# mir-group/pair_allegro

Measured on AMD Instinct MI355X. Metric: atom_steps_per_sec, higher is better.
Workload: dtype f32-equivalent (f16x2 split on the f16 matrix cores, f32 accumulate); 1 GPU; BASELINE config 4: 1000000-atom bulk Si (50^3 diamond cells), model S (l_max=1, U=32, S=64, 2 layers), r_max 5.0 A + skin 1.0 A, NVE dt=1 fs; grid=1x1x1, rebuilds=4, comm=serial, comm_transport=library/hosted/single-rank gather-scatter

## Files before the change

pair_allegro_amd/csrc/fused.hip:

```cpp
#include <hip/hip_runtime.h>

#include <cmath>
#include <algorithm>
#include <cstdio>
#include <cstdlib>
#include <cstring>
#include <type_traits>

#include "../../include/allegro_hip.h"
#include "engine.h"
#define AHIP_RING 4
#include "fused_common.h"
#include "fused_h.h"
#include "prims.h"

#ifndef AHIP_FUSED_PART
#define AHIP_FUSED_PART 0
#endif
namespace ahip {


[[maybe_unused]] static constexpr int MAX_TILE_SLOTS = 128;
static constexpr int MAXNL = 3;
static constexpr int STG_LD = 132;
// ... 150 lines not shown
      } else { prev0 = acc0; prev1 = acc1; }
    }
    __builtin_amdgcn_sched_barrier(0);
  }
  wp += NS * 256;
  pin_s(wp);
}
template <int RB> __device__ __forceinline__ void ring_prime_b(__amdgpu_buffer_rsrc_t W, int wp, int v16, u32x4 (&ring)[RB]) {
  int wo = wp * 4;
  pin_s(wo);
#pragma unroll
  for (int j = 0; j < RB; ++j) ring[j] = __builtin_bit_cast(u32x4, bload_w(W, v16 + (j & 3) * 1024, wo + (j >> 2) * 4096));
}

template <int NW, int NL> __device__ __forceinline__ void reduce_stage(const Lds<NW, NL> &lds, const int *aoff, float *dst, int na, float scale, int tid) {
  const int fidx = tid & 127;
  for (int a = tid >> 7; a < na; a += NW / 2) {
    const int s0 = aoff[a], s1 = aoff[a + 1];
    float acc0 = 0.f, acc1 = 0.f, acc2 = 0.f, acc3 = 0.f;
    int sl = s0;
    for (; sl + 4 <= s1; sl += 4) {
      acc0 += lds.stage[sl * STG_LD + fidx];
      acc1 += lds.stage[(sl + 1) * STG_LD + fidx];
      acc2 += lds.stage[(sl + 2) * STG_LD + fidx];
      acc3 += lds.stage[(sl + 3) * STG_LD + fidx];
    }
    for (; sl < s1; ++sl) acc0 += lds.stage[sl * STG_LD + fidx];
    dst[a * ENV_LD + fidx] = scale * ((acc0 + acc1) + (acc2 + acc3));
  }
}
enum { PH_GEOM = 0, PH_TB, PH_EMB, PH_ENV, PH_TP, PH_MIX, PH_LAT, PH_OUT, PH_BLAT, PH_BMIX, PH_BTP, PH_BENV, PH_BEMB, PH_BTB, PH_FIN, PH_N };
#define PHASE(id) do { if (PROF) { long long _t = clock64(); pacc[id] += _t - tprev; tprev = _t; } } while (0)

template <int AR> struct RingT {
  int act = 1;
  f32x4 f[AR != 0 ? 1 : RING];
  u32x4 b[AR == 0 ? 1 : (AR == 1 ? RINGB : AR == 2 ? RINGB2 : RINGH)];
};
template <int AR, int KT, int NT, bool ACC, int RPI, class Epi>
__device__ __forceinline__ void lin(__amdgpu_buffer_rsrc_t W, int &wp, const f32x4 (&in)[KT], f32x4 (&out)[NT], int v16, RingT<AR> &ring, Epi epi) {
  if (!ring.act) {
    if constexpr (!ACC) {
#pragma unroll
      for (int t = 0; t < NT; ++t) out[t] = f32x4{0.f, 0.f, 0.f, 0.f};
    }
    return;
  }
  if constexpr (AR == 3) {
    static_assert(KT % 2 == 0, "K-steps are pairs of 16-feature tiles");
    Hop b[1][KT / 2], unused[1][NT / 2];
#pragma unroll
    for (int ks = 0; ks < KT / 2; ++ks) b[0][ks] = split_pair_h(in[2 * ks], in[2 * ks + 1]);
    Epi ep[1] = {epi};
    linear_h<1, KT / 2, NT, ACC, false, (4 * RPI) % RINGH, Epi>(W, wp, b, reinterpret_cast<f32x4 (&)[1][NT]>(out), unused, v16, ring.b, ep);
  } else if constexpr (AR != 0) {
    static_assert(KT % 2 == 0, "K-steps are pairs of 16-feature tiles");
    constexpr int NTERM = AR == 1 ? 3 : 2;
    Bop b[KT / 2], unused[NT / 2];
#pragma unroll
    for (int ks = 0; ks < KT / 2; ++ks) b[ks] = split_pair(in[2 * ks], in[2 * ks + 1]);
    linear_b<KT / 2, NT, ACC, false, (2 * NTERM * RPI) % RingB<NTERM>::N, Epi, NTERM>(W, wp, b, out, unused, v16, ring.b, epi);
  } else {
    linear_s<KT, NT, ACC, (4 * RPI) % RING, Epi>(W, wp, in, out, v16, ring.f, epi);
  }
}

template <int RPI, class Epi>
__device__ __forceinline__ void lin_m3(__amdgpu_buffer_rsrc_t W, int &wp, const f32x4 (&in0)[2], const f32x4 (&in1)[2], const f32x4 (&in2)[2], f32x4 (&out)[3][2], int v16,
                                       RingT<3> &ring, Epi (&epi)[3]) {
  if (!ring.act) {
#pragma unroll
    for (int q = 0; q < 3; ++q) { out[q][0] = f32x4{0.f, 0.f, 0.f, 0.f}; out[q][1] = f32x4{0.f, 0.f, 0.f, 0.f}; }
    return;
  }
  Hop b[3][1], unused[3][1];
  b[0][0] = split_pair_h(in0[0], in0[1]); b[1][0] = split_pair_h(in1[0], in1[1]); b[2][0] = split_pair_h(in2[0], in2[1]);
  linear_h<3, 1, 2, false, false, (4 * RPI) % RINGH, Epi>(W, wp, b, out, unused, v16, ring.b, epi);
}

struct TileIn {
  int a0, a1, e0, e1;
  float rx, ry, rz;
  int eii, jat, tt;
  int eoff;
};
__device__ __forceinline__ void tile_fetch(const FusedArgs &A, int tile, int ntiles, int s, int tid, TileIn &n) {
  n.a0 = n.a1 = n.e0 = n.e1 = 0;
  n.rx = 1.f; n.ry = 0.f; n.rz = 0.f;
  n.eii = 0; n.jat = 0; n.tt = 0; n.eoff = 0;
  if (tile >= ntiles) return;
  n.a0 = A.tile_a0[tile]; n.a1 = A.tile_a0[tile + 1]; n.e0 = A.tile_e0[tile]; n.e1 = A.tile_e0[tile + 1];
  const int e = n.e0 + s, na = n.a1 - n.a0;
  if (e < n.e1) {
    n.rx = A.rvec[3 * (size_t)e]; n.ry = A.rvec[3 * (size_t)e + 1]; n.rz = A.rvec[3 * (size_t)e + 2];
    n.eii = A.e_ii[e];
    n.jat = A.e_j[e];
    n.tt = A.e_tt[e];
  }
  if (tid <= na) n.eoff = A.eoff[n.a0 + tid];
}

template <int NW, bool PROF, int AR, bool TBT, int NLT, int MD = 2, bool VA = false>
__global__ void __launch_bounds__(NW * 64, 2) k_fused(FusedArgs A) {
  constexpr int NTHREADS = NW * 64, MAXA = Lds<NW>::MAXA;
  constexpr bool SAVEZ = AR == 3;
  constexpr bool PARKV = true;
  constexpr bool STGROWS = true;
  constexpr int OZL = 4 + 4 * (MD - 1), OU = 4 + 4 * MD, OVIN = 8 + 4 * MD;
  static_assert(MD >= 1 && MD <= 3 && (MD == 2 || (AR == 3 && TBT)), "latent MLP depth 1 / 3: f16x2 instances with the two-body table only");
  __shared__ Lds<NW, NLT> lds;
  const int tid = threadIdx.x, lane = tid & 63, j = lane & 15, g = lane >> 4, wave = tid >> 6;
  const int v16 = lane * 16;
  __amdgpu_buffer_rsrc_t SB, WB;
  {
    unsigned long long b = (unsigned long long)(A.scratch + (size_t)blockIdx.x * A.wg_scratch + (size_t)wave * A.wave_scratch);
    unsigned lo = __builtin_amdgcn_readfirstlane((unsigned)b), hi = __builtin_amdgcn_readfirstlane((unsigned)(b >> 32));
    SB = __builtin_amdgcn_make_buffer_rsrc((void *)(((unsigned long long)hi << 32) | lo), 0, (int)(A.wave_scratch * 4), 0x00020000);
    WB = __builtin_amdgcn_make_buffer_rsrc((void *)A.wbase, 0, A.wbytes, 0x00020000);
  }
  if (A.maxdeg_sel && ((*A.maxdeg_sel <= 64) != (NW == 4))) return;
  const float *__restrict__ Wb = A.wbase;
  for (int k = tid; k < A.NL * 160; k += NTHREADS) {
    const int pth = (k % 160) / 32;
    lds.tp[k / 160][k % 160] = Wb[A.o_tpl + k] * (pth == 1 ? C_P1 : pth == 4 ? C_P4 : 1.f);
  }
  const int ntiles = *A.ntiles;
  constexpr int NL = NLT;
  double acc_part = 0.0;
  long long pacc[PH_N];
  long long tprev = 0;
  const long long t_clk0 = clock64(), t_wall0 = wall_clock64();
  if (PROF) {
#pragma unroll
    for (int k = 0; k < PH_N; ++k) pacc[k] = 0;
    tprev = clock64();
  }
  float *const pk = lds.park[wave];
  RingT<AR> ring;
  int wp = A.o_stream;
  if constexpr (AR != 0) ring_prime_b(WB, wp, v16, ring.b);
  else ring_prime(WB, wp, v16, ring.f);
  if (tid < MAXA) lds.eacc[tid] = 0.0;
  if (lane < 6) lds.virw[wave][lane] = 0.0;
  if (A.T <= 4 && tid < A.T * A.T) lds.rc[tid] = (float)A.rcut[tid];
  if (tid < A.T) { lds.scale[tid] = Wb[A.o_scale + tid]; lds.shift[tid] = Wb[A.o_shift + tid]; }
  if (tid < 2 * A.NL) lds.res[tid >> 1][tid & 1] = Wb[A.o_res[tid >> 1] + (tid & 1)];

  const int s = wave * 16 + j;
  float *const st = lds.stage + s * STG_LD;
  if (tid == 0) lds.chunk[0] = (int)atomicAdd(A.tile_counter, (unsigned)A.tchunk);
  __syncthreads();
  int par = 0, cpar = 0, ck = 0;
  int cbase = __builtin_amdgcn_readfirstlane(lds.chunk[0]);

  TileIn nx_;
  tile_fetch(A, cbase, ntiles, s, tid, nx_);

  for (;;) {
    const int tile = cbase + ck;
    if (tile >= ntiles) break;
    int claimed = 0;
    if (ck == 0 && tid == 0) claimed = (int)atomicAdd(A.tile_counter, (unsigned)A.tchunk);
    const int a0 = nx_.a0, a1 = nx_.a1, e0 = nx_.e0, e1 = nx_.e1;
    const int wact = __builtin_amdgcn_readfirstlane(e0 + wave * 16 < e1 ? 1 : 0);
    ring.act = wact;
    const int v16t = wact ? v16 : 0x7ffffff0;
    const int na = a1 - a0;
    par ^= 1;
    int *const aoffp = lds.aoff[par];
    const int e = e0 + s;
    const bool valid = e < e1;
    const float rx = nx_.rx, ry = nx_.ry, rz = nx_.rz;
    const int aloc = valid ? nx_.eii - a0 : 0, jat = nx_.jat, ti = nx_.tt >> 4, tj = nx_.tt & 15;
    if (tid <= na) aoffp[tid] = nx_.eoff - e0;
    const float d = sqrtf(rx * rx + ry * ry + rz * rz);
    const float inv = 1.f / d;
    const float nx = rx * inv, ny = ry * inv, nz = rz * inv;
    const float rc = A.T <= 4 ? lds.rc[ti * A.T + tj] : (float)A.rcut[ti * A.T + tj];
    const float xx = d / rc;
    float fc, dfc_dx;
    cutoff_poly_c(A.p, A.cp, xx, fc, dfc_dx);
    if (!valid) { fc = 0.f; dfc_dx = 0.f; }
    const float Y1 = C_S3 * ny, Y2 = C_S3 * nz, Y3 = C_S3 * nx;
    const float pref = 2.f / rc;
    const float PI = 3.14159265358979323846f;
    const float *const envrow = lds.env[0] + aloc * ENV_LD;
    const float *const denvrow = lds.denv + aloc * ENV_LD;
    PHASE(PH_GEOM);

    f32x4 x[4];
    float tb_t = 0.f, tb_invh = 0.f;
    if constexpr (TBT) {
      tb_invh = (float)A.tb_nk / rc;
      const float sft = d * tb_invh;
      const int kq = min((int)sft, A.tb_nk - 1);
      tb_t = sft - (float)kq;
#ifdef ABL_NOTBGATHER
      const int tb_off = (A.o_tbtab + 4 * g) * 4;
#else
      const int tb_off = (A.o_tbtab + ((ti * A.T + tj) * A.tb_nk + kq) * 256 + 4 * g) * 4;
#endif
      const float vm = (valid && xx < 1.f) ? 1.f : 0.f;
#pragma unroll
      for (int t = 0; t < 4; ++t) {
        const f32x4 c0 = bload_w(WB, tb_off + (t * 4 + 0) * 64, 0), c1 = bload_w(WB, tb_off + (t * 4 + 1) * 64, 0);
        const f32x4 c2 = bload_w(WB, tb_off + (t * 4 + 2) * 64, 0), c3 = bload_w(WB, tb_off + (t * 4 + 3) * 64, 0);
        x[t] = (c0 + tb_t * (c1 + tb_t * (c2 + tb_t * c3))) * vm;
        bstore(SB, v16t, (R_Z1TB() + t) * ROW * 4, (c1 + tb_t * (2.f * c2 + (3.f * tb_t) * c3)) * (vm * tb_invh));
      }
    } else {
      f32x4 z[4], z2[4];
      {
        const float *pt = Wb + A.o_pair + (size_t)(ti * A.T + tj) * 64;
#pragma unroll
        for (int t = 0; t < 4; ++t) z[t] = *(const f32x4 *)(pt + 16 * t + 4 * g);
      }
      f32x4 bfin[2];
#pragma unroll
      for (int r = 0; r < 4; ++r) {
        const float n = (float)(4 * g + r + 1);
        bfin[0][r] = g < 2 ? pref * __builtin_amdgcn_sinf(0.5f * n * xx) * inv * fc : 0.f;
        bfin[1][r] = 0.f;
      }
      lin<AR, 2, 4, true, 0>(WB, wp, bfin, z, v16t, ring, EpiSiluSaveD{SB, R_Z1TB(), v16t});
      lin<AR, 4, 4, false, 0>(WB, wp, z, z2, v16t, ring, EpiSiluSaveD{SB, R_Z2TB(), v16t});
      lin<AR, 4, 4, false, 0>(WB, wp, z2, x, v16t, ring, EpiSaveScale{{SB, R_U0(), v16t}, fc});
    }
    PHASE(PH_TB);
    {
      f32x4 w0[4];
      lin<AR, 4, 4, false, 0>(WB, wp, x, w0, v16t, ring, EpiSavePark{{SB, R_W0(), v16t}, pk, 0, lane});
    }
    if (ck == 0 && tid == 0) lds.chunk[cpar ^ 1] = claimed;
// ... 95 lines not shown
          if (stg && (H) >= MD - 1) { \
            if (SAVEZ && (H) == MD) lin<AR, KT, 4, false, 0>(WB, wp, IN, OUT, v16t, ring, EpiSiluSaveZL{sq, 4}); \
            else lin<AR, KT, 4, false, 0>(WB, wp, IN, OUT, v16t, ring, EpiSiluSaveDL{sq, (H) == MD ? 4 : 0}); \
          } else if (SAVEZ && (H) == MD) lin<AR, KT, 4, false, 0>(WB, wp, IN, OUT, v16t, ring, EpiSiluSaveZ{SB, RL + 4 * (H), v16t}); \
          else lin<AR, KT, 4, false, 0>(WB, wp, IN, OUT, v16t, ring, EpiSiluSaveD{SB, RL + 4 * (H), v16t}); } while (0)
        AHIP_HIDDEN(6, cat, z, 1);
        if constexpr (MD >= 2) AHIP_HIDDEN(4, z, z2, 2);
        if constexpr (MD >= 3) AHIP_HIDDEN(4, z2, z, 3);
#undef AHIP_HIDDEN
        f32x4 (&zl)[4] = MD == 2 ? z2 : z;
        const float ra = lds.res[kk][0], rbf = lds.res[kk][1] * fc;
        if (!last) {
          f32x4 xn[4];
          if constexpr (SAVEZ) lin<AR, 4, 4, false, 0>(WB, wp, zl, xn, v16t, ring, EpiResidualNS<4>{x, ra, rbf});
          else lin<AR, 4, 4, false, 0>(WB, wp, zl, xn, v16t, ring, EpiResidual<4>{{SB, RL + OU, v16t}, x, ra, rbf});
          x[0] = xn[0]; x[1] = xn[1]; x[2] = xn[2]; x[3] = xn[3];
        } else {
          f32x4 za[2], up[2];
          if constexpr (SAVEZ) lin<AR, 4, 2, false, 0>(WB, wp, zl, up, v16t, ring, EpiNone{});
          else lin<AR, 4, 2, false, 0>(WB, wp, zl, up, v16t, ring, EpiSave{SB, RL + OU, v16t});
          lin<AR, 4, 2, false, 0>(WB, wp, x, za, v16t, ring, EpiNone{});
          zr[0] = ra * za[0] + rbf * up[0]; zr[1] = ra * za[1] + rbf * up[1];
        }
      }
      PHASE(PH_LAT);
    }

    f32x4 upre[4], zt[4], w0h[2];
#pragma unroll
    for (int t = 0; t < 2; ++t) if (!SAVEZ) upre[t] = bload(SB, v16t, (R_LAYER(NL - 1, MD) + OU + t) * ROW * 4);
    if (!STGROWS) load_rows<4>(SB, R_LAYER(NL - 1, MD) + OZL, zt, v16t);
    __builtin_amdgcn_sched_barrier(0);
    f32x4 wo1[2];
#pragma unroll
    for (int t = 0; t < 2; ++t) wo1[t] = *(const f32x4 *)(Wb + A.o_out1 + 16 * t + 4 * g);
    float eps = 0.f;
#pragma unroll
    for (int t = 0; t < 2; ++t)
#pragma unroll
      for (int r = 0; r < 4; ++r) eps += silu1(zr[t][r]) * wo1[t][r];
    eps = gsum(eps);
    asm volatile("" : "+v"(eps));

    float bsc = 1.f;
    if constexpr (AR == 3) {
      int bex;
      (void)frexpf(lds.scale[ti] * A.cenv, &bex);
      bex = min(max(bex, -100), 100);
      bsc = ldexpf(1.f, -bex);
      if (g == 0) st[128] = ldexpf(1.f, bex);
    }
    const float deps = valid ? lds.scale[ti] * A.cenv * bsc : 0.f;
    f32x4 dx[4];
    f32x4 dzr[2];
#pragma unroll
    for (int t = 0; t < 2; ++t)
#pragma unroll
      for (int r = 0; r < 4; ++r) dzr[t][r] = deps * wo1[t][r] * dsilu1(zr[t][r]);
    lin<AR, 2, 4, false, 0>(WB, wp, dzr, dx, v16t, ring, EpiNone{});
    if (STGROWS) {
#pragma unroll
      for (int t = 0; t < 4; ++t) zt[t] = stg_load(st + 4 * g, 4 + t);
    }
    float dfc_part = 0.f, dY1 = 0.f, dY2 = 0.f, dY3 = 0.f;
    PHASE(PH_OUT);

#pragma unroll
    for (int kk = NL - 1; kk >= 0; --kk) {
// ... 249 lines not shown
      const float inve = 1.f / sqrtf(rxe * rxe + rye * rye + rze * rze);
      const float nxe = rxe * inve, nye = rye * inve, nze = rze * inve;
      const float gn = Gx * nxe + Gy * nye + Gz * nze;
      const float gx = dd * nxe + (Gx - gn * nxe) * inve;
      const float gy = dd * nye + (Gy - gn * nye) * inve;
      const float gz = dd * nze + (Gz - gn * nze) * inve;
      if (A.dbg && valid && g == 0) {
        float *dp = A.dbg + 8 * (size_t)e;
        dp[0] = gx; dp[1] = gy; dp[2] = gz; dp[3] = dd; dp[4] = dfc_tot; dp[5] = y1; dp[6] = y2; dp[7] = y3;
      }
#if !defined(ABL_NOW) && !defined(ABL_NOROWS) && !defined(ABL_NOROWLD) && !defined(ABL_NOROWST)
      if (AR == 3 && valid && !(fabsf(gx) + fabsf(gy) + fabsf(gz) + fabsf(eps) < 3.0e38f)) *A.err = 1;
#endif
      if (g == 0) {
        st[0] = valid ? gx : 0.f; st[1] = valid ? gy : 0.f; st[2] = valid ? gz : 0.f; st[3] = valid ? eps : 0.f;
        if (valid) {
#ifndef ABL_NOATOM
          atomicAdd(&A.f[3 * (size_t)jat], -(double)gx);
          atomicAdd(&A.f[3 * (size_t)jat + 1], -(double)gy);
          atomicAdd(&A.f[3 * (size_t)jat + 2], -(double)gz);
#endif
        }
      }
      float w6[6] = {-rx * gx, -ry * gy, -rz * gz, -0.5f * (rx * gy + ry * gx), -0.5f * (rx * gz + rz * gx), -0.5f * (ry * gz + rz * gy)};
#pragma unroll
      for (int c = 0; c < 6; ++c) w6[c] = valid ? w6[c] : 0.f;
#pragma unroll
      for (int c = 0; c < 6; ++c) {
#pragma unroll
        for (int off = 8; off > 0; off >>= 1) w6[c] += __shfl_xor(w6[c], off, 64);
      }
      if (lane < 6) {
        const float mine = lane == 0 ? w6[0] : lane == 1 ? w6[1] : lane == 2 ? w6[2] : lane == 3 ? w6[3] : lane == 4 ? w6[4] : w6[5];
        lds.virw[wave][lane] += (double)mine;
      }
      if constexpr (VA) vatom_scatter(A.vatom, jat, g, valid, rx, ry, rz, gx, gy, gz);
    }
    int tidf = tid;
    asm volatile("" : "+v"(tidf));
    const int caf = tidf >> 4;
    int2 cil = make_int2(0, 0);
    if (caf < na) cil = A.centre[a0 + caf];
    __syncthreads();
    {
      const int col = tidf & 3, part = (tidf >> 2) & 3;
      float sum = 0.f;
      if (caf < na)
        for (int sl = aoffp[caf] + part; sl < aoffp[caf + 1]; sl += 4) sum += lds.stage[sl * STG_LD + col];
      sum += __shfl_xor(sum, 4, 64);
      sum += __shfl_xor(sum, 8, 64);
      if (caf < na && part == 0) {
        if (col < 3) atomicAdd(&A.f[3 * (size_t)cil.x + col], (double)sum);
        else {
          const float ei = lds.scale[cil.y] * (sum * A.cenv) + lds.shift[cil.y];
          if (A.eatom) A.eatom[cil.x] = (double)ei;
          lds.eacc[caf] += (double)ei;
        }
      }
    }
    PHASE(PH_FIN);
    if (++ck == A.tchunk) { ck = 0; cpar ^= 1; cbase = __builtin_amdgcn_readfirstlane(lds.chunk[cpar]); }
  }
  __syncthreads();
  if (tid == 0) {
    for (int a = 0; a < MAXA; ++a) acc_part += lds.eacc[a];
  } else if (tid >= 64 && tid < 70) {
    for (int w = 0; w < NW; ++w) acc_part += lds.virw[w][tid - 64];
  }
  if (PROF && lane == 0) {
#pragma unroll
    for (int k = 0; k < PH_N; ++k) atomicAdd((unsigned long long *)&A.prof[k], (unsigned long long)pacc[k]);
  }
  if (A.prof && tid == 0) {
    long long *o = A.prof + PH_N + 4 * (size_t)blockIdx.x;
    o[0] = clock64() - t_clk0;
    o[1] = t_wall0;
    o[2] = wall_clock64();
    o[3] = ((long long)__builtin_amdgcn_s_getreg((20 << 0) | (0 << 6) | (31 << 11)) << 32) | (unsigned)__builtin_amdgcn_s_getreg((4 << 0) | (0 << 6) | (31 << 11));
  }
  if (tid == 0) A.partial[7 * (size_t)blockIdx.x] = acc_part;
  if (tid >= 64 && tid < 70) A.partial[7 * (size_t)blockIdx.x + 1 + (tid - 64)] = acc_part;
}


void fused_launch_bf16(int nw, bool prof, int arith, bool tbt, int grid, hipStream_t s, const FusedArgs &A);
void fused_launch_f16(int nw, bool prof, int md, int grid, hipStream_t s, const FusedArgs &A);
#if AHIP_FUSED_PART == 2
void fused_launch_f16(int nw, bool prof, int md, int grid, hipStream_t s, const FusedArgs &A) {
#ifdef AHIP_ASM_ONLY
#ifndef AHIP_ASM_NW
#define AHIP_ASM_NW 4
#endif
  hipLaunchKernelGGL((k_fused<AHIP_ASM_NW, false, 3, true, 2, 2>), dim3(grid), dim3(AHIP_ASM_NW * 64), 0, s, A);
#else
  dispatch<Choices<4, 8>, Choices<1, 2, 3>, Choices<1, 3, 2>, Variants>([&](auto nw, auto nl, auto md, auto var) {
    if constexpr (var != VAR_PROF || md == 2) hipLaunchKernelGGL((k_fused<nw, var == VAR_PROF, 3, true, nl, md, var == VAR_VA>), dim3(grid), dim3(nw * 64), 0, s, A);
  }, nw, A.NL, md, fused_variant(A.vatom, prof && md == 2));
#endif
}
#endif
#if AHIP_FUSED_PART == 1
void fused_launch_bf16(int nw, bool prof, int arith, bool tbt, int grid, hipStream_t s, const FusedArgs &A) {
  dispatch<Choices<4, 8>, Choices<1, 2>, Choices<1, 0>, Choices<1, 2, 3>, Variants>([&](auto nw, auto b3, auto tb, auto nl, auto var) {
    hipLaunchKernelGGL((k_fused<nw, var == VAR_PROF, b3, tb != 0, nl, 2, var == VAR_VA>), dim3(grid), dim3(nw * 64), 0, s, A);
  }, nw, arith, tbt, A.NL, fused_variant(A.vatom, prof));
}
#endif

#if AHIP_FUSED_PART == 0
struct FusedState {
  DevBuf wbuf, scratch;
  TileBufs tiles;
  FusedArgs args;
  bool ready = false, prof_on = false, dbg_on = false, clk_on = false;
  bool tbt = true;
  int md = 2;
  Arith arith = AR_F32;
  DevBuf prof, dbg;
  int ncu = 256;
  int force_nw = 0;
};

static inline unsigned bf16_trunc_bits(float f) { unsigned u; std::memcpy(&u, &f, 4); return u >> 16; }
static inline float bf16_bits_to_f(unsigned h) { unsigned u = h << 16; float f; std::memcpy(&f, &u, 4); return f; }
static int append_frag_b(std::vector<float> &out, const double *W, int K, int N, int ldw, int nterm = 3) {
  int KS, NT;
// ... 94 lines not shown
      const double *mx = T_(lk + ".mix");
      fwd(mx, 32, 32);
      for (int c = 0; c < (h2 ? 1 : 3); ++c) fwd(mx + 1024, 32, 32);
    }
    fwd(T_(lk + ".lat.w0"), 96, 64);
    for (int hl = 1; hl < MD; ++hl) fwd(T_(lk + ".lat.w" + std::to_string(hl)), 64, 64);
    if (k < NL - 1) fwd(T_(lk + ".lat.w" + std::to_string(MD)), 64, 64);
    else {
      fwd(w3r.data(), 64, 32);
      fwd(T_("out.w0"), 64, 32);
    }
  }
  bwd(T_("out.w0"), 64, 32);
  for (int k = NL - 1; k >= 0; --k) {
    const std::string lk = "l" + std::to_string(k + 1);
    if (k < NL - 1) bwd(T_(lk + ".lat.w" + std::to_string(MD)), 64, 64);
    else bwd(w3r.data(), 64, 32);
    for (int hl = MD - 1; hl >= 1; --hl) bwd(T_(lk + ".lat.w" + std::to_string(hl)), 64, 64);
    bwd(T_(lk + ".lat.w0"), 96, 64);
    if (k < NL - 1) {
      const double *mx = T_(lk + ".mix");
      bwd(mx, 32, 32);
      for (int c = 0; c < (h2 ? 1 : 3); ++c) bwd(mx + 1024, 32, 32);
    }
    bwd(T_(lk + ".env"), 64, 64);
  }
  bwd(T_("emb.w"), 64, 64);
  if (!tbt) {
    bwd(T_("tb.w2"), 64, 64);
    bwd(T_("tb.w1"), 64, 64);
    bwd(wc, 8, 64);
  }
  {
    const size_t n = (size_t)(st.arith == AR_BF16X3 ? RINGB : st.arith == AR_TF32EQ ? RINGB2 : h2 ? RINGH : RING) * 256;
    for (size_t i = 0; i < n; ++i) w.push_back(w[stream0 + i]);
  }
  st.ncu = fused_prepare_tail(m, h, w, A, st.wbuf, tbt, 5, 32, nullptr, st.arith, h_flags);
  A.wave_scratch = (long long)R_TOTAL(NL, MD) * ROW;
  st.scratch.reserve((size_t)st.ncu * 8 * A.wave_scratch * sizeof(float));
  A.scratch = st.scratch.as<float>();
  st.tiles.partial.reserve((size_t)st.ncu * 2 * 7 * sizeof(double));
  if (const char *nwe = std::getenv("AHIP_FUSED_NW")) st.force_nw = std::atoi(nwe);
  st.tiles.ntiles.reserve(64);
  st.prof.reserve((64 + 4 * 2 * (size_t)st.ncu) * sizeof(long long));
  const char *pe = std::getenv("AHIP_FUSED_PROF");
  st.prof_on = pe && pe[0] == '1';
  st.clk_on = std::getenv("AHIP_FUSED_CLK") != nullptr;
  const char *de = std::getenv("AHIP_FUSED_DBG");
  st.dbg_on = de && de[0] == '1';
  st.ready = true;
}

bool fused_run(Model &m, const ComputeArgs &a, std::string *why) {
  if (m.edges_T_size != 4) { if (why) *why = "edge vectors are not float32"; return false; }
  fused_prepare(m);
  FusedState &st = *m.fused_state;
  if (st.prof_on || st.clk_on || st.dbg_on) edges_counts(m);
  int nw = 0;
  if (!m.counts_pending) {
    if (m.last_max_deg > MAX_TILE_SLOTS) {
      if (why) *why = "an atom has " + std::to_string(m.last_max_deg) + " edges (> 128 per tile)";
      return false;
    }
    nw = m.last_max_deg <= 64 ? 4 : 8;
    if (st.force_nw == 8 || (st.force_nw == 4 && m.last_max_deg <= 64)) nw = st.force_nw;
  } else if (st.force_nw == 8) nw = 8;
  else if (m.max_list_row >= 0 && m.max_list_row <= 64) nw = 4;
// ... 105 lines not shown
      int n = feat16(t, r, g);
      if (n < N) out[row * N + n] = o[t][r];
    }
}

template <int KS, int NT, int NTERM>
__global__ void __launch_bounds__(128) k_selftest_linear_b(const float *Wf, int wbytes, const float *in, int K, float *out, int N) {
  const int lane = threadIdx.x & 63, j = lane & 15, g = lane >> 4, row = (threadIdx.x >> 6) * 16 + j;
  f32x4 a[2 * KS], o[NT];
#pragma unroll
  for (int t = 0; t < 2 * KS; ++t)
#pragma unroll
    for (int r = 0; r < 4; ++r) {
      int k = feat16(t, r, g);
      a[t][r] = k < K ? in[row * K + k] : 0.f;
    }
  Bop b[KS], ob[NT / 2];
#pragma unroll
  for (int ks = 0; ks < KS; ++ks) b[ks] = split_pair(a[2 * ks], a[2 * ks + 1]);
  __amdgpu_buffer_rsrc_t WB = __builtin_amdgcn_make_buffer_rsrc((void *)Wf, 0, wbytes, 0x00020000);
  u32x4 ring[RingB<NTERM>::N];
  int wp = 0;
  ring_prime_b(WB, wp, lane * 16, ring);
  linear_b<KS, NT, false, false, 0, EpiNone, NTERM>(WB, wp, b, o, ob, lane * 16, ring, EpiNone{});
#pragma unroll
  for (int t = 0; t < NT; ++t)
#pragma unroll
    for (int r = 0; r < 4; ++r) {
      int n = feat16(t, r, g);
      if (n < N) out[row * N + n] = o[t][r];
    }
}

template <int KS, int NT>
__global__ void __launch_bounds__(128) k_selftest_linear_h(const float *Wf, int wbytes, const float *in, int K, float *out, int N) {
  const int lane = threadIdx.x & 63, j = lane & 15, g = lane >> 4, row = (threadIdx.x >> 6) * 16 + j;
  f32x4 a[2 * KS], o[1][NT];
#pragma unroll
  for (int t = 0; t < 2 * KS; ++t)
#pragma unroll
    for (int r = 0; r < 4; ++r) {
      int k = feat16(t, r, g);
      a[t][r] = k < K ? in[row * K + k] : 0.f;
    }
  Hop b[1][KS], ob[1][NT / 2];
#pragma unroll
  for (int ks = 0; ks < KS; ++ks) b[0][ks] = split_pair_h(a[2 * ks], a[2 * ks + 1]);
  __amdgpu_buffer_rsrc_t WB = __builtin_amdgcn_make_buffer_rsrc((void *)Wf, 0, wbytes, 0x00020000);
  u32x4 ring[RINGH];
  int wp = 0;
  ring_prime_b(WB, wp, lane * 16, ring);
  EpiNone ep[1];
  linear_h<1, KS, NT, false, false, 0, EpiNone>(WB, wp, b, o, ob, lane * 16, ring, ep);
#pragma unroll
  for (int t = 0; t < NT; ++t)
#pragma unroll
    for (int r = 0; r < 4; ++r) {
      int n = feat16(t, r, g);
      if (n < N) out[row * N + n] = o[0][t][r];
    }
}

#endif
}

#if AHIP_FUSED_PART == 0
using namespace ahip;

extern "C" int ahip_debug_fused_edges(ahip_model *mh, float *out, long long nedges) {
  ahip::Model *m = (ahip::Model *)mh;
  if (!m || !m->fused_state) return AHIP_ERR_STATE;
  FusedState &st = *m->fused_state;
  if (!st.dbg_on || !st.dbg.p || nedges != m->nedges) return AHIP_ERR_STATE;
  if (hipDeviceSynchronize() != hipSuccess) return AHIP_ERR_DEVICE;
  try { copy_d2h(out, st.dbg.p, (size_t)nedges * 8 * sizeof(float)); } catch (...) { return AHIP_ERR_DEVICE; }
  return 0;
}

extern "C" int ahip_debug_fused_linear(int K, int N, const double *W, const float *in, float *out) {
  try {
    const char *ar = std::getenv("AHIP_FUSED_ARITH");
    const int nterm = (ar && std::string(ar) == "tf32eq") ? 2 : 3;
    const bool h2 = ar && std::string(ar) == "f16x2";
    const bool b3 = h2 || (ar && (std::string(ar) == "b3" || std::string(ar) == "bf16x3" || std::string(ar) == "tf32eq"));
    std::vector<float> frag;
    int KT, NT;
    if (h2) { append_frag_h(frag, W, K, N, N); frag_dims_b(K, N, KT, NT); }
    else if (b3) { append_frag_b(frag, W, K, N, N, nterm); frag_dims_b(K, N, KT, NT); }
    else { append_frag(frag, W, K, N, N); frag_dims(K, N, KT, NT); }
    frag.resize(frag.size() + (size_t)(RINGB + 2) * 256, 0.f);
    float *dW = nullptr, *din = nullptr, *dout = nullptr;
    AHIP_CHECK(hipMalloc((void **)&dW, frag.size() * sizeof(float)));
    AHIP_CHECK(hipMalloc((void **)&din, (size_t)32 * K * sizeof(float)));
    AHIP_CHECK(hipMalloc((void **)&dout, (size_t)32 * N * sizeof(float)));
    AHIP_CHECK(hipMemcpy(dW, frag.data(), frag.size() * sizeof(float), hipMemcpyHostToDevice));
    AHIP_CHECK(hipMemcpy(din, in, (size_t)32 * K * sizeof(float), hipMemcpyHostToDevice));
    bool ok = true;
    const int wbytes = (int)(frag.size() * sizeof(float));
#define CASEB(ks, nt) do { if (h2) hipLaunchKernelGGL((k_selftest_linear_h<ks, nt>), dim3(1), dim3(128), 0, 0, dW, wbytes, din, K, dout, N); \
                           else if (nterm == 3) hipLaunchKernelGGL((k_selftest_linear_b<ks, nt, 3>), dim3(1), dim3(128), 0, 0, dW, wbytes, din, K, dout, N); \
                           else hipLaunchKernelGGL((k_selftest_linear_b<ks, nt, 2>), dim3(1), dim3(128), 0, 0, dW, wbytes, din, K, dout, N); } while (0)
    if (b3) {
      if (KT == 1 && NT == 2) CASEB(1, 2);
      else if (KT == 1 && NT == 4) CASEB(1, 4);
      else if (KT == 2 && NT == 2) CASEB(2, 2);
      else if (KT == 2 && NT == 4) CASEB(2, 4);
      else if (KT == 3 && NT == 4) CASEB(3, 4);
      else if (KT == 2 && NT == 6) CASEB(2, 6);
      else ok = false;
    } else
#undef CASEB_
#define CASE(kt, nt) hipLaunchKernelGGL((k_selftest_linear<kt, nt>), dim3(1), dim3(128), 0, 0, dW, wbytes, din, K, dout, N)
    if (KT == 2 && NT == 2) CASE(2, 2);
    else if (KT == 2 && NT == 4) CASE(2, 4);
    else if (KT == 4 && NT == 2) CASE(4, 2);
    else if (KT == 4 && NT == 4) CASE(4, 4);
    else if (KT == 6 && NT == 4) CASE(6, 4);
    else if (KT == 4 && NT == 6) CASE(4, 6);
    else ok = false;
#undef CASE
    if (ok) {
      AHIP_CHECK(hipDeviceSynchronize());
      AHIP_CHECK(hipMemcpy(out, dout, (size_t)32 * N * sizeof(float), hipMemcpyDeviceToHost));
    }
    (void)hipFree(dW); (void)hipFree(din); (void)hipFree(dout);
    return ok ? 0 : AHIP_ERR_UNSUPPORTED;
  } catch (const std::exception &) { return AHIP_ERR_DEVICE; }
}
#endif
```

pair_allegro_amd/csrc/fused_h.h:

```cpp
#pragma once
#include <cstring>

#include "fused_common.h"

namespace ahip {

typedef _Float16 f16x2 __attribute__((ext_vector_type(2)));
typedef _Float16 f16x8 __attribute__((ext_vector_type(8)));
typedef float f32x2 __attribute__((ext_vector_type(2)));
struct Hop { u32x4 hi, lo; };
static constexpr float H_LO_SCALE = 2048.f, H_LO_INV = 1.f / 2048.f;
static constexpr int RINGH = 8;

__device__ __forceinline__ f32x4 mfma_h(u32x4 a, u32x4 b, f32x4 c) {
  return __builtin_amdgcn_mfma_f32_16x16x32_f16(__builtin_bit_cast(f16x8, a), __builtin_bit_cast(f16x8, b), c, 0, 0, 0);
}
__device__ __forceinline__ void split2_h(float v0, float v1, unsigned &hi, unsigned &lo) {
  const f32x2 v = {v0, v1};
  const f16x2 h = __builtin_convertvector(v, f16x2);
  const f32x2 r = (v - __builtin_convertvector(h, f32x2)) * H_LO_SCALE;
  const f16x2 l = __builtin_convertvector(r, f16x2);
  hi = __builtin_bit_cast(unsigned, h);
  lo = __builtin_bit_cast(unsigned, l);
}
__device__ __forceinline__ Hop split_pair_h(const f32x4 &t0, const f32x4 &t1) {
  Hop b;
  unsigned h, l;
  split2_h(t0[0], t0[1], h, l); b.hi[0] = h; b.lo[0] = l;
  split2_h(t0[2], t0[3], h, l); b.hi[1] = h; b.lo[1] = l;
  split2_h(t1[0], t1[1], h, l); b.hi[2] = h; b.lo[2] = l;
  split2_h(t1[2], t1[3], h, l); b.hi[3] = h; b.lo[3] = l;
  return b;
}

__device__ __forceinline__ void ring_prime_h(__amdgpu_buffer_rsrc_t W, int wp, int v16, u32x4 (&ring)[RINGH]) {
  int wo = wp * 4;
  pin_s(wo);
#pragma unroll
  for (int j = 0; j < RINGH; ++j) ring[j] = __builtin_bit_cast(u32x4, bload_w(W, v16 + (j & 3) * 1024, wo + (j >> 2) * 4096));
}

template <class E> __device__ __forceinline__ auto epi_apply2(E &e, int ot, int r, f32x2 v, int) -> decltype(e.apply2(ot, r, v)) { return e.apply2(ot, r, v); }
template <class E> __device__ __forceinline__ f32x2 epi_apply2(E &e, int ot, int r, f32x2 v, long) { return f32x2{e.apply(ot, r, v[0]), e.apply(ot, r + 1, v[1])}; }

template <int G, int KS, int NT, bool ACC, bool SPLIT, int RP, class Epi>
__device__ __forceinline__ void linear_h(__amdgpu_buffer_rsrc_t W, int &wp, const Hop (&in)[G][KS], f32x4 (&out)[G][NT], Hop (&outb)[G][NT / 2],
                                         int v16, u32x4 (&ring)[RINGH], Epi (&epi)[G]) {
  static_assert(NT % 2 == 0, "output tiles are processed in pairs");
  constexpr int RB = RINGH, NF = 4, NP = NT / 2, NSTEP = NP * KS, NS = NF * NSTEP;
  constexpr int MF = 6 * G;
  f32x4 ah[G][2], ac[G][2], prev[G][2];
  int wo = (wp + RB * 256) * 4;
  pin_s(wo);
#pragma unroll
  for (int s = 0; s < NSTEP; ++s) {
    const int p = s / KS, ks = s % KS;
    if (ks == 0) {
#pragma unroll
      for (int g = 0; g < G; ++g)
#pragma unroll
        for (int hh = 0; hh < 2; ++hh) {
          ah[g][hh] = ACC ? out[g][2 * p + hh] : f32x4{0.f, 0.f, 0.f, 0.f};
          ac[g][hh] = f32x4{0.f, 0.f, 0.f, 0.f};
        }
    }
    u32x4 a[NF];
#pragma unroll
    for (int i = 0; i < NF; ++i) {
      a[i] = ring[(RP + NF * s + i) % RB];
      ring[(RP + NF * s + i) % RB] = __builtin_bit_cast(u32x4, bload_w(W, v16 + i * 1024, wo));
    }
    wo += NF * 1024;
    pin_s(wo);
#pragma unroll
    for (int m = 0; m < 3; ++m) {
#pragma unroll
      for (int hh = 0; hh < 2; ++hh) {
#pragma unroll
        for (int g = 0; g < G; ++g) {
          if (m == 0) ac[g][hh] = mfma_h(a[2 + hh], in[g][ks].hi, ac[g][hh]);
          else if (m == 1) ac[g][hh] = mfma_h(a[hh], in[g][ks].lo, ac[g][hh]);
          else ah[g][hh] = mfma_h(a[hh], in[g][ks].hi, ah[g][hh]);
          if (p > 0) {
            const int idx = ks * MF + (m * 2 + hh) * G + g, tot = KS * MF, NE = 4 * G;
            const int e0 = (idx * NE + tot - 1) / tot, e1 = ((idx + 1) * NE + tot - 1) / tot;
#pragma unroll
            for (int e = 0; e < NE; ++e)
              if (e >= e0 && e < e1) {
                const int eg = e / 4, th = (e % 4) / 2, r = 2 * (e % 2), ot = 2 * (p - 1) + th;
                const f32x2 y = epi_apply2(epi[eg], ot, r, f32x2{prev[eg][th][r], prev[eg][th][r + 1]}, 0);
                out[eg][ot][r] = y[0]; out[eg][ot][r + 1] = y[1];
                if (e % 4 == 3) {
                  epi[eg].flush(2 * (p - 1));
                  if (SPLIT) outb[eg][p - 1] = split_pair_h(out[eg][2 * (p - 1)], out[eg][2 * (p - 1) + 1]);
                }
              }
          }
          __builtin_amdgcn_sched_barrier(0);
        }
      }
    }
    if (ks == KS - 1) {
#pragma unroll
      for (int g = 0; g < G; ++g) {
        const f32x4 r0 = ac[g][0] * H_LO_INV + ah[g][0], r1 = ac[g][1] * H_LO_INV + ah[g][1];
        epi[g].tile_done(2 * p, r0);
        epi[g].tile_done(2 * p + 1, r1);
        if (p == NP - 1) {
#pragma unroll
          for (int r = 0; r < 4; r += 2) {
            const f32x2 y0 = epi_apply2(epi[g], 2 * p, r, f32x2{r0[r], r0[r + 1]}, 0), y1 = epi_apply2(epi[g], 2 * p + 1, r, f32x2{r1[r], r1[r + 1]}, 0);
            out[g][2 * p][r] = y0[0]; out[g][2 * p][r + 1] = y0[1]; out[g][2 * p + 1][r] = y1[0]; out[g][2 * p + 1][r + 1] = y1[1];
          }
          epi[g].flush(2 * p);
          if (SPLIT) outb[g][p] = split_pair_h(out[g][2 * p], out[g][2 * p + 1]);
        } else { prev[g][0] = r0; prev[g][1] = r1; }
      }
    }
    __builtin_amdgcn_sched_barrier(0);
  }
  wp += NS * 256;
  pin_s(wp);
}

static void frag_dims_b(int K, int N, int &KS, int &NT) {
  KS = (K + 31) / 32;
  NT = (N + 15) / 16;
  NT += NT & 1;
}
// ... 35 lines not shown
```

Measured before the change: 28.36 million atom-steps/s.

## Deepen f16x2 weight ring to 12 with deferred, cross-call fragment refills

```diff
diff --git a/pair_allegro_amd/csrc/fused.hip b/pair_allegro_amd/csrc/fused.hip
--- a/pair_allegro_amd/csrc/fused.hip
+++ b/pair_allegro_amd/csrc/fused.hip
@@ -206,13 +206,30 @@
 enum { PH_GEOM = 0, PH_TB, PH_EMB, PH_ENV, PH_TP, PH_MIX, PH_LAT, PH_OUT, PH_BLAT, PH_BMIX, PH_BTP, PH_BENV, PH_BEMB, PH_BTB, PH_FIN, PH_N };
 #define PHASE(id) do { if (PROF) { long long _t = clock64(); pacc[id] += _t - tprev; tprev = _t; } } while (0)
 
+template <int AR> struct RingMem {};
 template <int AR> struct RingT {
   int act = 1;
   f32x4 f[AR != 0 ? 1 : RING];
-  u32x4 b[AR == 0 ? 1 : (AR == 1 ? RINGB : AR == 2 ? RINGB2 : RINGH)];
+  u32x4 b[AR == 0 ? 1 : (AR == 1 ? RINGB : RINGB2)];
+  __device__ explicit RingT(RingMem<AR> &) {}
 };
+template <> struct RingMem<3> { u32x4 b[RINGH3]; };
+template <> struct RingT<3> {
+  int act = 1;
+  int cnt = 0, tile_nf = 0;
+  bool pend = false;
+  u32x4 (&b)[RINGH3];
+  __device__ explicit RingT(RingMem<3> &m) : b(m.b) {}
+};
+__host__ __device__ constexpr int h_tile_frags(int NL, int MD) { return 16 + 32 * NL * (3 + MD); }
 template <int AR, int KT, int NT, bool ACC, int RPI, class Epi>
 __device__ __forceinline__ void lin(__amdgpu_buffer_rsrc_t W, int &wp, const f32x4 (&in)[KT], f32x4 (&out)[NT], int v16, RingT<AR> &ring, Epi epi) {
+  int c0 = 0;
+  bool pend = false, defer = false;
+  if constexpr (AR == 3) {
+    c0 = ring.cnt; ring.cnt += KT * NT;
+    pend = ring.pend; defer = ring.cnt != ring.tile_nf; ring.pend = defer;
+  }
   if (!ring.act) {
     if constexpr (!ACC) {
 #pragma unroll
@@ -226,7 +243,7 @@
 #pragma unroll
     for (int ks = 0; ks < KT / 2; ++ks) b[0][ks] = split_pair_h(in[2 * ks], in[2 * ks + 1]);
     Epi ep[1] = {epi};
-    linear_h<1, KT / 2, NT, ACC, false, (4 * RPI) % RINGH, Epi>(W, wp, b, reinterpret_cast<f32x4 (&)[1][NT]>(out), unused, v16, ring.b, ep);
+    linear_h<1, KT / 2, NT, ACC, false, 0, Epi, RINGH3>(W, wp, b, reinterpret_cast<f32x4 (&)[1][NT]>(out), unused, v16, ring.b, ep, c0, ring.tile_nf, pend, defer);
   } else if constexpr (AR != 0) {
     static_assert(KT % 2 == 0, "K-steps are pairs of 16-feature tiles");
     constexpr int NTERM = AR == 1 ? 3 : 2;
@@ -242,6 +259,10 @@
 template <int RPI, class Epi>
 __device__ __forceinline__ void lin_m3(__amdgpu_buffer_rsrc_t W, int &wp, const f32x4 (&in0)[2], const f32x4 (&in1)[2], const f32x4 (&in2)[2], f32x4 (&out)[3][2], int v16,
                                        RingT<3> &ring, Epi (&epi)[3]) {
+  const int c0 = ring.cnt;
+  ring.cnt += 4;
+  const bool pend = ring.pend, defer = true;
+  ring.pend = defer;
   if (!ring.act) {
 #pragma unroll
     for (int q = 0; q < 3; ++q) { out[q][0] = f32x4{0.f, 0.f, 0.f, 0.f}; out[q][1] = f32x4{0.f, 0.f, 0.f, 0.f}; }
@@ -249,7 +270,7 @@
   }
   Hop b[3][1], unused[3][1];
   b[0][0] = split_pair_h(in0[0], in0[1]); b[1][0] = split_pair_h(in1[0], in1[1]); b[2][0] = split_pair_h(in2[0], in2[1]);
-  linear_h<3, 1, 2, false, false, (4 * RPI) % RINGH, Epi>(W, wp, b, out, unused, v16, ring.b, epi);
+  linear_h<3, 1, 2, false, false, 0, Epi, RINGH3>(W, wp, b, out, unused, v16, ring.b, epi, c0, ring.tile_nf, pend, defer);
 }
 
 struct TileIn {
@@ -282,6 +303,7 @@
   constexpr bool STGROWS = true;
   constexpr int OZL = 4 + 4 * (MD - 1), OU = 4 + 4 * MD, OVIN = 8 + 4 * MD;
   static_assert(MD >= 1 && MD <= 3 && (MD == 2 || (AR == 3 && TBT)), "latent MLP depth 1 / 3: f16x2 instances with the two-body table only");
+  static_assert(AR != 3 || TBT, "f16x2: h_tile_frags counts the stream of the two-body table instances");
   __shared__ Lds<NW, NLT> lds;
   const int tid = threadIdx.x, lane = tid & 63, j = lane & 15, g = lane >> 4, wave = tid >> 6;
   const int v16 = lane * 16;
@@ -310,7 +332,8 @@
     tprev = clock64();
   }
   float *const pk = lds.park[wave];
-  RingT<AR> ring;
+  RingMem<AR> ring_mem;
+  RingT<AR> ring(ring_mem);
   int wp = A.o_stream;
   if constexpr (AR != 0) ring_prime_b(WB, wp, v16, ring.b);
   else ring_prime(WB, wp, v16, ring.f);
@@ -336,8 +359,9 @@
     int claimed = 0;
     if (ck == 0 && tid == 0) claimed = (int)atomicAdd(A.tile_counter, (unsigned)A.tchunk);
     const int a0 = nx_.a0, a1 = nx_.a1, e0 = nx_.e0, e1 = nx_.e1;
-    const int wact = __builtin_amdgcn_readfirstlane(e0 + wave * 16 < e1 ? 1 : 0);
+    const int wact = __builtin_amdgcn_readfirstlane(e0 + (AR == 3 ? __builtin_amdgcn_readfirstlane(wave) : wave) * 16 < e1 ? 1 : 0);
     ring.act = wact;
+    if constexpr (AR == 3) { ring.cnt = 0; ring.tile_nf = h_tile_frags(NLT, MD); ring.pend = false; }
     const int v16t = wact ? v16 : 0x7ffffff0;
     const int na = a1 - a0;
     par ^= 1;
@@ -368,11 +392,13 @@
       tb_invh = (float)A.tb_nk / rc;
       const float sft = d * tb_invh;
       const int kq = min((int)sft, A.tb_nk - 1);
+      int gq = tid;
+      if constexpr (AR == 3) asm volatile("" : "+v"(gq));
       tb_t = sft - (float)kq;
 #ifdef ABL_NOTBGATHER
       const int tb_off = (A.o_tbtab + 4 * g) * 4;
 #else
-      const int tb_off = (A.o_tbtab + ((ti * A.T + tj) * A.tb_nk + kq) * 256 + 4 * g) * 4;
+      const int tb_off = (A.o_tbtab + ((ti * A.T + tj) * A.tb_nk + kq) * 256 + 4 * (AR == 3 ? (gq >> 4) & 3 : g)) * 4;
 #endif
       const float vm = (valid && xx < 1.f) ? 1.f : 0.f;
 #pragma unroll
@@ -534,8 +560,10 @@
     if (!STGROWS) load_rows<4>(SB, R_LAYER(NL - 1, MD) + OZL, zt, v16t);
     __builtin_amdgcn_sched_barrier(0);
     f32x4 wo1[2];
-#pragma unroll
-    for (int t = 0; t < 2; ++t) wo1[t] = *(const f32x4 *)(Wb + A.o_out1 + 16 * t + 4 * g);
+    int gro = tid;
+    if constexpr (AR == 3) asm volatile("" : "+v"(gro));
+#pragma unroll
+    for (int t = 0; t < 2; ++t) wo1[t] = *(const f32x4 *)(Wb + A.o_out1 + 16 * t + 4 * (AR == 3 ? (gro >> 4) & 3 : g));
     float eps = 0.f;
 #pragma unroll
     for (int t = 0; t < 2; ++t)
@@ -851,7 +879,9 @@
       }
       if (lane < 6) {
         const float mine = lane == 0 ? w6[0] : lane == 1 ? w6[1] : lane == 2 ? w6[2] : lane == 3 ? w6[3] : lane == 4 ? w6[4] : w6[5];
-        lds.virw[wave][lane] += (double)mine;
+        int tidv = tid;
+        if constexpr (AR == 3) asm volatile("" : "+v"(tidv));
+        lds.virw[AR == 3 ? tidv >> 6 : wave][AR == 3 ? tidv & 63 : lane] += (double)mine;
       }
       if constexpr (VA) vatom_scatter(A.vatom, jat, g, valid, rx, ry, rz, gx, gy, gz);
     }
@@ -881,6 +911,9 @@
     if (++ck == A.tchunk) { ck = 0; cpar ^= 1; cbase = __builtin_amdgcn_readfirstlane(lds.chunk[cpar]); }
   }
   __syncthreads();
+  int tid_ = threadIdx.x;
+  if constexpr (AR == 3) asm volatile("" : "+v"(tid_));
+#define tid tid_
   if (tid == 0) {
     for (int a = 0; a < MAXA; ++a) acc_part += lds.eacc[a];
   } else if (tid >= 64 && tid < 70) {
@@ -899,6 +932,7 @@
   }
   if (tid == 0) A.partial[7 * (size_t)blockIdx.x] = acc_part;
   if (tid >= 64 && tid < 70) A.partial[7 * (size_t)blockIdx.x + 1 + (tid - 64)] = acc_part;
+#undef tid
 }
 
 
@@ -910,7 +944,13 @@
 #ifndef AHIP_ASM_NW
 #define AHIP_ASM_NW 4
 #endif
-  hipLaunchKernelGGL((k_fused<AHIP_ASM_NW, false, 3, true, 2, 2>), dim3(grid), dim3(AHIP_ASM_NW * 64), 0, s, A);
+#ifndef AHIP_ASM_NL
+#define AHIP_ASM_NL 2
+#endif
+#ifndef AHIP_ASM_MD
+#define AHIP_ASM_MD 2
+#endif
+  hipLaunchKernelGGL((k_fused<AHIP_ASM_NW, false, 3, true, AHIP_ASM_NL, AHIP_ASM_MD>), dim3(grid), dim3(AHIP_ASM_NW * 64), 0, s, A);
 #else
   dispatch<Choices<4, 8>, Choices<1, 2, 3>, Choices<1, 3, 2>, Variants>([&](auto nw, auto nl, auto md, auto var) {
     if constexpr (var != VAR_PROF || md == 2) hipLaunchKernelGGL((k_fused<nw, var == VAR_PROF, 3, true, nl, md, var == VAR_VA>), dim3(grid), dim3(nw * 64), 0, s, A);
@@ -1071,7 +1111,7 @@
     bwd(wc, 8, 64);
   }
   {
-    const size_t n = (size_t)(st.arith == AR_BF16X3 ? RINGB : st.arith == AR_TF32EQ ? RINGB2 : h2 ? RINGH : RING) * 256;
+    const size_t n = (size_t)(st.arith == AR_BF16X3 ? RINGB : st.arith == AR_TF32EQ ? RINGB2 : h2 ? RINGH3 : RING) * 256;
     for (size_t i = 0; i < n; ++i) w.push_back(w[stream0 + i]);
   }
   st.ncu = fused_prepare_tail(m, h, w, A, st.wbuf, tbt, 5, 32, nullptr, st.arith, h_flags);
@@ -1243,33 +1283,44 @@
     }
 }
 
-template <int KS, int NT>
+template <int KS, int NT, int G, int PH>
 __global__ void __launch_bounds__(128) k_selftest_linear_h(const float *Wf, int wbytes, const float *in, int K, float *out, int N) {
-  const int lane = threadIdx.x & 63, j = lane & 15, g = lane >> 4, row = (threadIdx.x >> 6) * 16 + j;
-  f32x4 a[2 * KS], o[1][NT];
-#pragma unroll
-  for (int t = 0; t < 2 * KS; ++t)
-#pragma unroll
-    for (int r = 0; r < 4; ++r) {
-      int k = feat16(t, r, g);
-      a[t][r] = k < K ? in[row * K + k] : 0.f;
-    }
-  Hop b[1][KS], ob[1][NT / 2];
-#pragma unroll
-  for (int ks = 0; ks < KS; ++ks) b[0][ks] = split_pair_h(a[2 * ks], a[2 * ks + 1]);
+  const int lane = threadIdx.x & 63, j = lane & 15, g = lane >> 4, wv = threadIdx.x >> 6;
+  f32x4 o[G][NT];
+  Hop b[G][KS], ob[G][NT / 2];
+#pragma unroll
+  for (int q = 0; q < G; ++q) {
+    const int row = ((wv + q) & 1) * 16 + j;
+    f32x4 a[2 * KS];
+#pragma unroll
+    for (int t = 0; t < 2 * KS; ++t)
+#pragma unroll
+      for (int r = 0; r < 4; ++r) {
+        int k = feat16(t, r, g);
+        a[t][r] = k < K ? in[row * K + k] : 0.f;
+      }
+#pragma unroll
+    for (int ks = 0; ks < KS; ++ks) b[q][ks] = split_pair_h(a[2 * ks], a[2 * ks + 1]);
+  }
   __amdgpu_buffer_rsrc_t WB = __builtin_amdgcn_make_buffer_rsrc((void *)Wf, 0, wbytes, 0x00020000);
-  u32x4 ring[RINGH];
-  int wp = 0;
-  ring_prime_b(WB, wp, lane * 16, ring);
-  EpiNone ep[1];
-  linear_h<1, KS, NT, false, false, 0, EpiNone>(WB, wp, b, o, ob, lane * 16, ring, ep);
-#pragma unroll
-  for (int t = 0; t < NT; ++t)
-#pragma unroll
-    for (int r = 0; r < 4; ++r) {
-      int n = feat16(t, r, g);
-      if (n < N) out[row * N + n] = o[0][t][r];
-    }
+  u32x4 ring[RINGH3];
+#pragma unroll
+  for (int jf = 0; jf < RINGH3; ++jf)
+    ring[jf] = __builtin_bit_cast(u32x4, bload_w(WB, lane * 16, (jf < PH ? jf + RINGH3 : jf) * 1024));
+  int wp = PH * 256;
+  EpiNone ep[G];
+  linear_h<G, KS, NT, false, false, 0, EpiNone, RINGH3>(WB, wp, b, o, ob, lane * 16, ring, ep, PH, 0);
+#pragma unroll
+  for (int q = 0; q < G; ++q) {
+    const int row = ((wv + q) & 1) * 16 + j;
+#pragma unroll
+    for (int t = 0; t < NT; ++t)
+#pragma unroll
+      for (int r = 0; r < 4; ++r) {
+        int n = feat16(t, r, g);
+        if (n < N) out[(size_t)q * 32 * N + row * N + n] = o[q][t][r];
+      }
+  }
 }
 
 #endif
@@ -1292,27 +1343,37 @@
   try {
     const char *ar = std::getenv("AHIP_FUSED_ARITH");
     const int nterm = (ar && std::string(ar) == "tf32eq") ? 2 : 3;
-    const bool h2 = ar && std::string(ar) == "f16x2";
+    const bool h3 = ar && std::string(ar) == "f16x2g3";
+    const bool h2 = h3 || (ar && std::string(ar) == "f16x2");
     const bool b3 = h2 || (ar && (std::string(ar) == "b3" || std::string(ar) == "bf16x3" || std::string(ar) == "tf32eq"));
     std::vector<float> frag;
     int KT, NT;
-    if (h2) { append_frag_h(frag, W, K, N, N); frag_dims_b(K, N, KT, NT); }
+    constexpr int HPH = 8;
+    if (h2) { frag.assign((size_t)HPH * 256, 0.f); append_frag_h(frag, W, K, N, N); frag_dims_b(K, N, KT, NT); }
     else if (b3) { append_frag_b(frag, W, K, N, N, nterm); frag_dims_b(K, N, KT, NT); }
     else { append_frag(frag, W, K, N, N); frag_dims(K, N, KT, NT); }
     frag.resize(frag.size() + (size_t)(RINGB + 2) * 256, 0.f);
     float *dW = nullptr, *din = nullptr, *dout = nullptr;
     AHIP_CHECK(hipMalloc((void **)&dW, frag.size() * sizeof(float)));
     AHIP_CHECK(hipMalloc((void **)&din, (size_t)32 * K * sizeof(float)));
-    AHIP_CHECK(hipMalloc((void **)&dout, (size_t)32 * N * sizeof(float)));
+    const size_t nout = (size_t)32 * N, ncopy = h2 ? 9 : 1;
+    AHIP_CHECK(hipMalloc((void **)&dout, ncopy * nout * sizeof(float)));
+    AHIP_CHECK(hipMemset(dout, 0, ncopy * nout * sizeof(float)));
     AHIP_CHECK(hipMemcpy(dW, frag.data(), frag.size() * sizeof(float), hipMemcpyHostToDevice));
     AHIP_CHECK(hipMemcpy(din, in, (size_t)32 * K * sizeof(float), hipMemcpyHostToDevice));
-    bool ok = true;
+    bool ok = true, same = true;
     const int wbytes = (int)(frag.size() * sizeof(float));
-#define CASEB(ks, nt) do { if (h2) hipLaunchKernelGGL((k_selftest_linear_h<ks, nt>), dim3(1), dim3(128), 0, 0, dW, wbytes, din, K, dout, N); \
+#define CASEH(ks, nt, g, ph) hipLaunchKernelGGL((k_selftest_linear_h<ks, nt, g, ph>), dim3(1), dim3(128), 0, 0, dW + (HPH - ph) * 256, wbytes - (HPH - ph) * 1024, din, K, \
+                                                dout + (ph / 4) * 3 * nout, N)
+#define CASEB(ks, nt) do { if (h2) { CASEH(ks, nt, 1, 0); CASEH(ks, nt, 1, 4); CASEH(ks, nt, 1, 8); } \
                            else if (nterm == 3) hipLaunchKernelGGL((k_selftest_linear_b<ks, nt, 3>), dim3(1), dim3(128), 0, 0, dW, wbytes, din, K, dout, N); \
                            else hipLaunchKernelGGL((k_selftest_linear_b<ks, nt, 2>), dim3(1), dim3(128), 0, 0, dW, wbytes, din, K, dout, N); } while (0)
-    if (b3) {
+    if (h3) {
+      if (KT == 1 && NT == 2) { CASEH(1, 2, 3, 0); CASEH(1, 2, 3, 4); CASEH(1, 2, 3, 8); }
+      else ok = false;
+    } else if (b3) {
       if (KT == 1 && NT == 2) CASEB(1, 2);
+      else if (KT == 3 && NT == 2) CASEB(3, 2);
       else if (KT == 1 && NT == 4) CASEB(1, 4);
       else if (KT == 2 && NT == 2) CASEB(2, 2);
       else if (KT == 2 && NT == 4) CASEB(2, 4);
@@ -1332,9 +1393,17 @@
 #undef CASE
     if (ok) {
       AHIP_CHECK(hipDeviceSynchronize());
-      AHIP_CHECK(hipMemcpy(out, dout, (size_t)32 * N * sizeof(float), hipMemcpyDeviceToHost));
+      AHIP_CHECK(hipMemcpy(out, dout, nout * sizeof(float), hipMemcpyDeviceToHost));
+      if (h2) {
+        std::vector<float> all(ncopy * nout);
+        AHIP_CHECK(hipMemcpy(all.data(), dout, all.size() * sizeof(float), hipMemcpyDeviceToHost));
+        for (int ph = 0; ph < 3; ++ph)
+          for (int q = 0; q < (h3 ? 3 : 1); ++q)
+            if (std::memcmp(all.data() + ((size_t)ph * 3 + q) * nout, all.data(), nout * sizeof(float)) != 0) same = false;
+      }
     }
     (void)hipFree(dW); (void)hipFree(din); (void)hipFree(dout);
+    if (ok && !same) return AHIP_ERR_STATE;
     return ok ? 0 : AHIP_ERR_UNSUPPORTED;
   } catch (const std::exception &) { return AHIP_ERR_DEVICE; }
 }
diff --git a/pair_allegro_amd/csrc/fused_h.h b/pair_allegro_amd/csrc/fused_h.h
--- a/pair_allegro_amd/csrc/fused_h.h
+++ b/pair_allegro_amd/csrc/fused_h.h
@@ -11,6 +11,7 @@
 struct Hop { u32x4 hi, lo; };
 static constexpr float H_LO_SCALE = 2048.f, H_LO_INV = 1.f / 2048.f;
 static constexpr int RINGH = 8;
+static constexpr int RINGH3 = 12;
 
 __device__ __forceinline__ f32x4 mfma_h(u32x4 a, u32x4 b, f32x4 c) {
   return __builtin_amdgcn_mfma_f32_16x16x32_f16(__builtin_bit_cast(f16x8, a), __builtin_bit_cast(f16x8, b), c, 0, 0, 0);
@@ -43,15 +44,26 @@
 template <class E> __device__ __forceinline__ auto epi_apply2(E &e, int ot, int r, f32x2 v, int) -> decltype(e.apply2(ot, r, v)) { return e.apply2(ot, r, v); }
 template <class E> __device__ __forceinline__ f32x2 epi_apply2(E &e, int ot, int r, f32x2 v, long) { return f32x2{e.apply(ot, r, v[0]), e.apply(ot, r + 1, v[1])}; }
 
-template <int G, int KS, int NT, bool ACC, bool SPLIT, int RP, class Epi>
+template <int G, int KS, int NT, bool ACC, bool SPLIT, int RP, class Epi, int RB = RINGH>
 __device__ __forceinline__ void linear_h(__amdgpu_buffer_rsrc_t W, int &wp, const Hop (&in)[G][KS], f32x4 (&out)[G][NT], Hop (&outb)[G][NT / 2],
-                                         int v16, u32x4 (&ring)[RINGH], Epi (&epi)[G]) {
+                                         int v16, u32x4 (&ring)[RB], Epi (&epi)[G], const int c0 = 0, const int tile_nf = 0, const bool pend = false, const bool defer = false) {
   static_assert(NT % 2 == 0, "output tiles are processed in pairs");
-  constexpr int RB = RINGH, NF = 4, NP = NT / 2, NSTEP = NP * KS, NS = NF * NSTEP;
+  static_assert(RB == RINGH || (RB == RINGH3 && RP == 0), "ring depth 8 (phase RP) or 12 (phase from c0)");
+  constexpr int NF = 4, NP = NT / 2, NSTEP = NP * KS, NS = NF * NSTEP;
   constexpr int MF = 6 * G;
   f32x4 ah[G][2], ac[G][2], prev[G][2];
   int wo = (wp + RB * 256) * 4;
   pin_s(wo);
+  if constexpr (RB == RINGH3) {
+    if (pend) {
+#pragma unroll
+      for (int q = 0; q < NF; ++q) {
+        const int i = q ^ 2, c = c0 - NF + i, f = c + RB;
+        const int d = (tile_nf > 0 && f >= tile_nf) ? (tile_nf + c % RB - f) * 1024 : 0;
+        ring[c % RB] = __builtin_bit_cast(u32x4, bload_w(W, v16 + i * 1024, wo - NF * 1024 + d));
+      }
+    }
+  }
 #pragma unroll
   for (int s = 0; s < NSTEP; ++s) {
     const int p = s / KS, ks = s % KS;
@@ -65,22 +77,29 @@
         }
     }
     u32x4 a[NF];
+    if constexpr (RB == RINGH) {
 #pragma unroll
-    for (int i = 0; i < NF; ++i) {
-      a[i] = ring[(RP + NF * s + i) % RB];
-      ring[(RP + NF * s + i) % RB] = __builtin_bit_cast(u32x4, bload_w(W, v16 + i * 1024, wo));
+      for (int i = 0; i < NF; ++i) {
+        a[i] = ring[(RP + NF * s + i) % RB];
+        ring[(RP + NF * s + i) % RB] = __builtin_bit_cast(u32x4, bload_w(W, v16 + i * 1024, wo));
+      }
+      wo += NF * 1024;
+      pin_s(wo);
     }
-    wo += NF * 1024;
-    pin_s(wo);
+    const int cs = c0 + NF * s;
+    auto frag = [&](int i) -> u32x4 {
+      if constexpr (RB == RINGH) return a[i];
+      else return ring[(cs + i) % RB];
+    };
 #pragma unroll
     for (int m = 0; m < 3; ++m) {
 #pragma unroll
       for (int hh = 0; hh < 2; ++hh) {
 #pragma unroll
         for (int g = 0; g < G; ++g) {
-          if (m == 0) ac[g][hh] = mfma_h(a[2 + hh], in[g][ks].hi, ac[g][hh]);
-          else if (m == 1) ac[g][hh] = mfma_h(a[hh], in[g][ks].lo, ac[g][hh]);
-          else ah[g][hh] = mfma_h(a[hh], in[g][ks].hi, ah[g][hh]);
+          if (m == 0) ac[g][hh] = mfma_h(frag(2 + hh), in[g][ks].hi, ac[g][hh]);
+          else if (m == 1) ac[g][hh] = mfma_h(frag(hh), in[g][ks].lo, ac[g][hh]);
+          else ah[g][hh] = mfma_h(frag(hh), in[g][ks].hi, ah[g][hh]);
           if (p > 0) {
             const int idx = ks * MF + (m * 2 + hh) * G + g, tot = KS * MF, NE = 4 * G;
             const int e0 = (idx * NE + tot - 1) / tot, e1 = ((idx + 1) * NE + tot - 1) / tot;
@@ -95,6 +114,18 @@
                   if (SPLIT) outb[eg][p - 1] = split_pair_h(out[eg][2 * (p - 1)], out[eg][2 * (p - 1) + 1]);
                 }
               }
+          }
+          if constexpr (RB == RINGH3) {
+            if (hh == 1 && g == G - 1 && m != 1) {
+              if (!(defer && s == NSTEP - 1))
+#pragma unroll
+              for (int i = (m == 0 ? 2 : 0); i < (m == 0 ? 4 : 2); ++i) {
+                const int c = cs + i, f = c + RB;
+                const int d = (tile_nf > 0 && f >= tile_nf) ? (tile_nf + c % RB - f) * 1024 : 0;
+                ring[c % RB] = __builtin_bit_cast(u32x4, bload_w(W, v16 + i * 1024, wo + d));
+              }
+              if (m == 2) { wo += NF * 1024; pin_s(wo); }
+            }
           }
           __builtin_amdgcn_sched_barrier(0);
         }
```

After: 28.56 million atom-steps/s, median of 6. About the same (+0.7%).
